# CFD-Xing/gpu-benchmarking

Hardware: AMD Instinct MI355X
Metric: GDOF/s for 3D hex sum-factorisation, fp64, nq=2..10 sweep (higher is better)
Workload: dtype f64

## Files before the change

gpu-benchmarking_amd/__init__.py:

```python
from . import capi, logfmt, shard
from .bwdtrans import (
    bwdtrans_hex, bwdtrans_quad, sumsq, fill_sincos, fill_basis, fill_random, fill_l2norm,
    stream_copy, device_info, interleave64, bwdtrans_hex_interleaved, fill_vecadd, vector_add, fill_matvec, matvec, hex_wsp_doubles, quad_wsp_doubles, VARIANTS,
    specialise, specialisation_state, specialise_log, bwdtrans_specialised,
    iproduct_hex, iproduct_quad, bwdtrans_autograd, mass_hex, mass_quad,
    helmholtz_hex, helmholtz_quad, affine_helmholtz_hex, affine_helmholtz_quad,
    physderiv_hex, physderiv_quad,
    iprodderiv_hex, iprodderiv_quad, physderiv_autograd,
    diag_tables, diag_helmholtz_hex, diag_helmholtz_quad,
    GsMap, gs_setup, global_to_local, assemble, gs,
)
```

gpu-benchmarking_amd/bwdtrans.py:

```python
import collections
import ctypes

import torch

from . import capi

VARIANTS = {"auto": 0, "wave": 1, "thread": 2, "block-lds": 3, "block-glb": 4, "generic": 5,
            "mfma": 6, "mfma4": 7, "wave-rt": 8}


def _stream(stream, device=None):
    if stream is None:
        stream = torch.cuda.current_stream(device)
    return ctypes.c_void_p(stream.cuda_stream)


def _check_operands(what, operands, inp, lam=None):
    for name, t, need, optional in operands:
        if t is None and optional:
            if lam is not None and lam != 0.0:
                raise ValueError(f"{what}: {name}=None needs lam == 0")
            continue
        if not isinstance(t, torch.Tensor):
            raise TypeError(f"{what}: {name} must be a tensor")
        if t.numel() != need:
            raise ValueError(f"{what}: {name} has {t.numel()} values, not {need}")
        if t.dtype != inp.dtype:
            raise ValueError(f"{what}: {name} is {t.dtype}, in is {inp.dtype}")
        if t.device != inp.device:
            raise ValueError(f"{what}: {name} is on {t.device}, in is on {inp.device}")


def _dev_ptr(t, name, dtype=torch.float64):
    if not (isinstance(t, torch.Tensor) and t.is_cuda and t.dtype == dtype and t.is_contiguous()):
        raise TypeError(f"{name} must be a contiguous {dtype} CUDA/HIP tensor")
    return ctypes.c_void_p(t.data_ptr())


def _variant(v):
    return VARIANTS[v] if isinstance(v, str) else int(v)

# ... 568 lines not shown
```

gpu-benchmarking_amd/csrc/bwdtrans_hex.hip:

```cpp
#include "sf_dispatch.h"
#include "wave_launch.h"
#include "wave_table.h"

#include <cstdlib>

namespace sf
{

template <int NQ> struct HexSmall
{
    static constexpr int EC  = HexCfg<NQ>::EC == 1 ? 1
                               : ((HexCfg<NQ>::EC / 4 + 1) / 2 * 2 < 2 ? 2 : (HexCfg<NQ>::EC / 4 + 1) / 2 * 2);
    static constexpr int OUT = HexCfg<NQ>::OUT;
};

__global__ __launch_bounds__(256) void hex_nq2_stream_kernel(const double *__restrict__ b0,
                                                             const double *__restrict__ b1,
                                                             const double *__restrict__ b2,
                                                             const double *__restrict__ in,
                                                             double *__restrict__ out, uint64_t nelmt)
{
    constexpr int U   = 1;
    const uint64_t nv = nelmt * 4;
    const double c0 = b0[0], c1 = b0[1];
    double2_t *out2 = reinterpret_cast<double2_t *>(out);
    const uint64_t base = logical_block<64>() * (256ull * U) + threadIdx.x;
#pragma unroll
    for (int u = 0; u < U; ++u)
    {
        const uint64_t v = base + (uint64_t)u * 256;
        if (v < nv)
        {
            const int p    = (int)(v & 3);
            const double x = in[v >> 2];
            const double bj = b1[p & 1], bk = b2[p >> 1];
            const double2_t r = {((x * c0) * bj) * bk, ((x * c1) * bj) * bk};
            __builtin_nontemporal_store(r, out2 + v);
        }
    }
}

template <int NQ> static int go(const HexArgs &a, hipStream_t s)
{
    if constexpr (NQ == 2)
        return launch_stream(hex_nq2_stream_kernel, a.nelmt * 4, s, a.b0, a.b1, a.b2, a.in, a.out, a.nelmt);
    using C = HexCfg<NQ>;
    constexpr uint64_t per_block = (uint64_t)C::EC * C::WPB * (C::KM > 0 ? C::KM : 1);
    if (a.nelmt < 2 * per_block * (uint64_t)device_info().num_cu)
        return launch_hex_wave<NQ, HexSmall<NQ>::EC, 1, C::BM, C::MW, 1, HexSmall<NQ>::OUT>(a, s);
    constexpr uint64_t piece = hex_piece(NQ);
    if (piece > 0 && a.nelmt > 2 * piece)
    {
        static_assert(piece == 0 || piece % (8 * 64 * per_block) == 0, "pieces hold whole XCD windows");
        constexpr uint64_t NMT = (uint64_t)(NQ - 1) * (NQ - 1) * (NQ - 1), NQT = (uint64_t)NQ * NQ * NQ;
        for (uint64_t lo = 0; lo < a.nelmt; lo += piece)
        {
            HexArgs part = a;
            part.in      = a.in + lo * NMT;
            part.out     = a.out + lo * NQT;
            part.nelmt   = a.nelmt - lo < piece ? a.nelmt - lo : piece;
            const int rc = launch_hex_wave<NQ, C::EC, C::WPB, C::BM, C::MW, C::KM, C::OUT, C::MF>(part, s);
            if (rc != SF_OK)
                return rc;
        }
        return SF_OK;
    }
    return launch_hex_wave<NQ, C::EC, C::WPB, C::BM, C::MW, C::KM, C::OUT, C::MF>(a, s);
}

template <> int launch_bwd_wave<3, double>(unsigned nq, const HexArgs &a, hipStream_t s)
{
    switch (nq)
    {
    case 2: return go<2>(a, s);
    case 3: return go<3>(a, s);
    case 4: return go<4>(a, s);
    case 5: return go<5>(a, s);
    case 6: return go<6>(a, s);
    case 7: return go<7>(a, s);
    case 8: return go<8>(a, s);
    case 9: return go<9>(a, s);
    case 10: return go<10>(a, s);
    case 11: return go<11>(a, s);
    default: return SF_ENOTBUILT;
    }
}

template <int NQ> static int go_mfma(const HexArgs &a, hipStream_t s)
{
    if constexpr (NQ <= 10)
        return launch_hex_mfma<NQ, 2, 2, 2, 1>(a, s);
    else
    {
        constexpr int WPB = NQ == 11 ? 4 : 1;
        constexpr int MW  = (NQ == 14 || NQ == 15) ? 2 : 1;
        return launch_hex_mfma<NQ, 1, WPB, MW, 1, 64>(a, s);
    }
}

template <> int launch_bwd_mfma<3, double>(unsigned nq, const HexArgs &a, hipStream_t s)
// ... 119 lines not shown
```

gpu-benchmarking_amd/csrc/bwdtrans_quad.hip:

```cpp
#include "sf_dispatch.h"
#include "wave_launch.h"
#include "wave_table.h"

#include <cstdlib>

namespace sf
{

template <int NQ> struct QuadSmall
{
    static constexpr int EC = (QuadCfg<NQ>::EC / 4 + 1) / 2 * 2 < 2 ? 2 : (QuadCfg<NQ>::EC / 4 + 1) / 2 * 2;
};

__global__ __launch_bounds__(256) void quad_nq2_stream_kernel(const double *__restrict__ b0,
                                                              const double *__restrict__ b1,
                                                              const double *__restrict__ in,
                                                              double *__restrict__ out, uint64_t nelmt)
{
    constexpr int U   = 1;
    const uint64_t nv = nelmt * 2;
    const double c0 = b0[0], c1 = b0[1];
    double2_t *out2 = reinterpret_cast<double2_t *>(out);
    const uint64_t base = logical_block<64>() * (256ull * U) + threadIdx.x;
#pragma unroll
    for (int u = 0; u < U; ++u)
    {
        const uint64_t v = base + (uint64_t)u * 256;
        if (v < nv)
        {
            const double x  = in[v >> 1];
            const double bj = b1[v & 1];
            const double2_t r = {(x * c0) * bj, (x * c1) * bj};
            __builtin_nontemporal_store(r, out2 + v);
        }
    }
}

template <int NQ> static int go(const QuadArgs &a, hipStream_t s)
{
    if constexpr (NQ == 2)
        return launch_stream(quad_nq2_stream_kernel, a.nelmt * 2, s, a.b0, a.b1, a.in, a.out, a.nelmt);
    using C = QuadCfg<NQ>;
    constexpr uint64_t per_block = (uint64_t)C::EC * C::WPB * (C::KM > 0 ? C::KM : 1);
    if (a.nelmt < 2 * per_block * (uint64_t)device_info().num_cu)
        return launch_quad_wave<NQ, QuadSmall<NQ>::EC, 1, C::BM, C::MW, 1, C::OUT>(a, s);
    return launch_quad_wave<NQ, C::EC, C::WPB, C::BM, C::MW, C::KM, C::OUT, C::MF>(a, s);
}

typedef float float4_t __attribute__((ext_vector_type(4)));
__global__ __launch_bounds__(256) void quad_nq2_stream_f32_kernel(const float *__restrict__ b0, const float *__restrict__ b1,
                                                                  const float *__restrict__ in, float *__restrict__ out,
                                                                  uint64_t nelmt)
{
    const uint64_t v = logical_block<64>() * 256ull + threadIdx.x;
    if (v < nelmt)
    {
        const float x  = in[v];
        const float x0 = x * b0[0], x1 = x * b0[1];
        const float4_t r = {x0 * b1[0], x1 * b1[0], x0 * b1[1], x1 * b1[1]};
        __builtin_nontemporal_store(r, reinterpret_cast<float4_t *>(out) + v);
    }
}

constexpr int kQuadF32MfmaFrom = 25;

template <int NQ> static int go_f32(const QuadArgsT<float> &a, hipStream_t s)
{
    if constexpr (NQ == 2)
        return launch_stream(quad_nq2_stream_f32_kernel, a.nelmt, s, a.b0, a.b1, a.in, a.out, a.nelmt);
    if constexpr (NQ >= kQuadF32MfmaFrom)
    {
        constexpr int best = NQ == 25 ? 3 : ((NQ == 28 || NQ == 32) ? 2 : ((NQ == 26 || NQ == 30 || NQ == 31) ? 4 : (NQ == 27 ? 0 : 1)));
        static const int cfg = getenv("SF_F32_MFMA_CFG") ? atoi(getenv("SF_F32_MFMA_CFG")) : best;
        switch (cfg)
        {
        case 1: return launch_quad_mfma<NQ, 2, 4, 4, 2, (NQ != 32), 64, float>(a, s);
        case 2: return launch_quad_mfma<NQ, 4, 4, 2, 1, (NQ != 32), 64, float>(a, s);
        case 3: return launch_quad_mfma<NQ, 4, 4, 4, 1, (NQ != 32), 64, float>(a, s);
        case 4: return launch_quad_mfma<NQ, 2, 4, 4, 1, (NQ != 32), 64, float>(a, s);
// ... 114 lines not shown
```

gpu-benchmarking_amd/csrc/bwdtrans_wave.h:

```cpp
#pragma once

#include "sf_common.h"

namespace sf
{

enum OutMode
{
    OUT_ST8  = 0,
    OUT_ST16 = 1,
    OUT_LDS  = 2
};

enum BasisMode
{
    BASIS_LDS = 0,
    BASIS_SMEM = 1,
    BASIS_SMEM_COLS = 2,
    BASIS_SMEM_COLS16 = 3
};

template <typename T> struct VecOf
{
    static constexpr int W = 16 / (int)sizeof(T);
// ... 44 lines not shown
    static constexpr int SLAB_W1 = P1 * S1;
    static constexpr int SLAB_W2 = (DIM == 3) ? P2 * S2 : 0;
    static constexpr int SLAB0   = CMax<CMax<SLAB_IN, SLAB_W1>::value, SLAB_W2>::value;
    static constexpr int OUT_DBL = EC * OUT_ELEM;
    static constexpr int SLAB_NOOUT = (SLAB0 + VW - 1) / VW * VW;
    static constexpr int SLAB_OUT   = (CMax<SLAB0, OUT_DBL>::value + VW - 1) / VW * VW;
    static constexpr int SLAB       = SLAB_OUT;
    static constexpr int NLD  = VEC2 ? cdiv(IN_DBL / VW, kWave) : cdiv(IN_DBL, kWave);
    static constexpr bool ALIGN_OK = VEC2 && cdiv(IN_DBL / VW + 7, kWave) == NLD;
};

template <int DIM, int EC, typename T, int NQ0, int NQ1, int NQ2 = 2>
using BwdGeom = SweepGeom<DIM, EC, T, NQ0 - 1, NQ0, NQ1 - 1, NQ1, DIM == 3 ? NQ2 - 1 : 1, DIM == 3 ? NQ2 : 1>;

template <int NQ, int EC, int DIM, typename T = double> struct WaveGeom : BwdGeom<DIM, EC, T, NQ, NQ, NQ>
{
    static constexpr int NM  = NQ - 1;
    static constexpr int NMP = NM | 1;
    static constexpr int NMT = WaveGeom::IN_ELEM;
    static constexpr int NQT = WaveGeom::OUT_ELEM;
    static constexpr int NBAS = (NM * NQ + WaveGeom::VW - 1) / WaveGeom::VW * WaveGeom::VW;
};

template <class G, int WPB> constexpr size_t slab_lds_bytes()
{
    return sizeof(typename G::Scalar) * (size_t)WPB * G::SLAB;
}

__device__ __forceinline__ int align_shift(const void *p)
{
    return __builtin_amdgcn_readfirstlane((int)(((uintptr_t)p >> 4) & 7));
}

template <class G, int OUTM> constexpr int slab_doubles()
{
    return OUTM == OUT_LDS ? G::SLAB_OUT : G::SLAB_NOOUT;
}

template <int NQ, int EC, int DIM, int WPB, int BMODE, int OUTM, typename T = double>
constexpr size_t wave_lds_bytes()
{
    using G = WaveGeom<NQ, EC, DIM, T>;
    return sizeof(T) *
           (size_t)((BMODE == BASIS_LDS ? DIM * G::NBAS : 0) + WPB * slab_doubles<G, OUTM>());
}

struct ChunkIter
{
    uint64_t first, step, count;
};

template <int KMAP, int WPB, int XG = 0>
__device__ __forceinline__ ChunkIter chunk_iter(uint64_t nchunk, int wib)
{
    const uint64_t gw = logical_block<XG>() * WPB + wib;
    ChunkIter it;
    if constexpr (KMAP == 0)
    {
        const uint64_t nwave = (uint64_t)gridDim.x * WPB;
        it.first = gw;
        it.step  = nwave;
        it.count = gw < nchunk ? (nchunk - gw + nwave - 1) / nwave : 0;
    }
    else if constexpr (KMAP > 0)
    {
        it.first = gw * KMAP;
        it.step  = 1;
        it.count = it.first < nchunk ? (nchunk - it.first < KMAP ? nchunk - it.first : KMAP) : 0;
    }
    else
    {
        constexpr int K     = -KMAP;
        const uint64_t base = logical_block<XG>() * WPB * K;
        it.first            = base + wib;
        it.step             = WPB;
        const uint64_t end  = base + (uint64_t)WPB * K < nchunk ? base + (uint64_t)WPB * K : nchunk;
        it.count            = it.first < end ? (end - it.first + WPB - 1) / WPB : 0;
// ... 122 lines not shown
                if constexpr (G::IN_STRIDE == G::IN_LEN)
                {
                    *reinterpret_cast<V *>(slab + VW * v) = st[k];
                }
                else
                {
#pragma unroll
                    for (int j = 0; j < VW; ++j)
                    {
                        const int f          = VW * v + j;
                        slab[f + f / G::IN_LEN] = st[k][j];
                    }
                }
            }
        }
    }
    else
    {
#pragma unroll
        for (int k = 0; k < word_grid_regs<G::IN_DBL, typename G::Scalar>(); ++k)
#pragma unroll
            for (int h = 0; h < VW; ++h)
            {
                const int f = VW * (k * kWave + lane) - sh + h;
                if (f >= 0 && f < G::IN_DBL)
                {
                    if constexpr (G::IN_STRIDE == G::IN_LEN)
                        slab[f] = st[k][h];
                    else
                        slab[f + f / G::IN_LEN] = st[k][h];
                }
            }
    }
}

typedef float float2_t __attribute__((ext_vector_type(2)));
template <int NB, int N0, int NOUT, int NPASS>
__device__ __forceinline__ void fma_row(bool first, const double (&um)[NPASS], const double (&b)[NB],
                                        double (&acc)[NPASS][NOUT])
{
#pragma unroll
    for (int n = 0; n < NB; ++n)
#pragma unroll
        for (int s = 0; s < NPASS; ++s)
            acc[s][N0 + n] = first ? um[s] * b[n] : fma_t(um[s], b[n], acc[s][N0 + n]);
}
template <int NB, int N0, int NOUT, int NPASS>
__device__ __forceinline__ void fma_row(bool first, const float (&um)[NPASS], const float (&b)[NB],
                                        float (&acc)[NPASS][NOUT])
{
    constexpr int NPAIR = (NOUT >= 9 && NOUT <= 24) ? NB / 2 : 0;
#pragma unroll
    for (int n = 0; n < 2 * NPAIR; n += 2)
#pragma unroll
        for (int s = 0; s < NPASS; ++s)
        {
            const float2_t uu = {um[s], um[s]}, bb = {b[n], b[n + 1]};
            const float2_t a  = {acc[s][N0 + n], acc[s][N0 + n + 1]};
            const float2_t r  = first ? uu * bb : __builtin_elementwise_fma(uu, bb, a);
            acc[s][N0 + n]     = r.x;
            acc[s][N0 + n + 1] = r.y;
        }
#pragma unroll
    for (int n = 2 * NPAIR; n < NB; ++n)
#pragma unroll
        for (int s = 0; s < NPASS; ++s)
// ... 280 lines not shown
                if (d0 + h >= 0 && d0 + h < nvalid)
                    v[h] = src[d0 + h];
        }
        x[k] = v;
    }
#pragma unroll
    for (int k = 0; k < NW; ++k)
#pragma unroll
        for (int h = 0; h < VW; ++h)
        {
            const int f = VW * (k * NT + (int)threadIdx.x) - a + h;
            if (f >= 0 && f < NB)
            {
                const int w = f / G::IN_DBL, r = f - w * G::IN_DBL;
                T *dst      = slab0 + w * SLAB;
                if constexpr (G::IN_STRIDE == G::IN_LEN)
                    dst[r] = x[k][h];
                else
                    dst[r + r / G::IN_LEN] = x[k][h];
            }
        }
}

template <int NQ, int EC, int WPB, int BMODE, int MINW, int KMAP, int OUTM, int MEMF = 0,
          typename T = double>
__global__ __launch_bounds__(kWave *WPB, MINW) void hex_wave_kernel(
    const T *__restrict__ b0, const T *__restrict__ b1, const T *__restrict__ b2,
    const T *__restrict__ in, T *__restrict__ out, uint64_t nelmt)
{
    using G          = WaveGeom<NQ, EC, 3, T>;
    constexpr int NM = G::NM, NMP = G::NMP, NQ2 = NQ * NQ;
    static_assert(OUTM != OUT_ST16 || (NQ % 2 == 0 && sizeof(T) == 8),
                  "paired 16-byte stores need even nq and fp64");
    constexpr int SLAB = slab_doubles<G, OUTM>();

    extern __shared__ __attribute__((aligned(16))) unsigned char lds_raw[];
    T *lds = reinterpret_cast<T *>(lds_raw);
    const int lane = threadIdx.x & (kWave - 1);
    const int wib  = __builtin_amdgcn_readfirstlane(threadIdx.x >> 6);
    const T *const gb[3] = {b0, b1, b2};
    const T *bs[3];
    T *slab = wave_setup<G, 3, WPB, BMODE, SLAB>(lds, gb, bs, wib);

    constexpr int XG  = (MEMF >> 4) & 0xfff;
    constexpr bool BL = ((MEMF >> 16) & 1) != 0;
    static_assert(!BL || (KMAP == 1 && BMODE != BASIS_LDS), "cooperative input: one chunk per wave, basis in SGPRs");
    const uint64_t nchunk = (nelmt + EC - 1) / EC;
    const ChunkIter it    = chunk_iter<KMAP, WPB, XG>(nchunk, wib);
    if constexpr (BL)
    {
        const uint64_t first = logical_block<XG>() * (uint64_t)(WPB * EC);
        if (first < nelmt)
        {
            const uint64_t left = nelmt - first;
            block_load_stage<G, WPB, SLAB>(lds, in + first * G::NMT,
                                           left >= (uint64_t)(WPB * EC) ? WPB * G::IN_DBL : (int)left * G::NMT);
        }
        __syncthreads();
    }
    if (it.count == 0)
        return;

    constexpr bool AL = (MEMF & 4) && G::ALIGN_OK;
    typename G::Vec st[BL ? 1 : G::NLD];
    if constexpr (!BL)
        chunk_fetch<G, EC, !(MEMF & 1), AL>(st, in, it.first, nelmt, lane);

    uint64_t c = it.first;
    for (uint64_t n = 0; n < it.count; ++n, c += it.step)
    {
        const uint64_t left = nelmt - c * EC;
        const int evalid    = left >= EC ? EC : (int)left;

        if constexpr (!BL)
        {
            chunk_stage<G, AL>(st, slab, lane,
                               G::VEC2 ? (AL ? align_shift(in + c * G::IN_DBL) : 0)
                                       : line_offset<T>(in + c * G::IN_DBL));
            wave_lds_fence();

            if (n + 1 < it.count)
                chunk_fetch<G, EC, !(MEMF & 1), AL>(st, in, c + it.step, nelmt, lane);
        }

#define SWEEP G::Sw0
#define SWEEP_CONTRACT contract
#define SWEEP_BASIS bs[0]
#include "frag/sweep.inc"
#define SWEEP G::Sw1
#define SWEEP_CONTRACT contract
#define SWEEP_BASIS bs[1]
#include "frag/sweep.inc"
        {
            T u[G::PASS2][NM], acc[G::PASS2][NQ];
            read_pencils<NM, G::PASS2, G::P2, NMP>(u, slab, lane);
            contract<NM, NQ, G::PASS2, BMODE>(u, acc, bs[2]);
            T *oc = out + c * (uint64_t)(EC * G::NQT);
            if constexpr (OUTM == OUT_LDS)
            {
#define SWEEP G::Sw2
#include "frag/sweep_store.inc"
                chunk_flush<G, !(MEMF & 2), (MEMF & 8) != 0>(slab, oc, evalid * G::NQT, lane);
            }
            else
            {
#pragma unroll
                for (int s = 0; s < G::PASS2; ++s)
                {
                    const int t = s * kWave + lane;
                    const int e = t / NQ2, pl = t - e * NQ2;
                    if (((s + 1) * kWave <= G::P2 || t < G::P2) && e < evalid)
                        store_column<NQ, NQ2, OUTM == OUT_ST16, !(MEMF & 2)>(
                            acc[s], oc + e * G::NQT + pl, lane);
                }
            }
            wave_lds_fence();
        }
    }
}

template <int NQ, int EC, int WPB, int BMODE, int MINW, int KMAP, int OUTM, int MEMF = 0,
          typename T = double>
__global__ __launch_bounds__(kWave *WPB, MINW) void quad_wave_kernel(
    const T *__restrict__ b0, const T *__restrict__ b1, const T *__restrict__ in,
    T *__restrict__ out, uint64_t nelmt)
{
    using G          = WaveGeom<NQ, EC, 2, T>;
    constexpr int NM = G::NM, NMP = G::NMP;
    static_assert(OUTM != OUT_ST16 || (NQ % 2 == 0 && sizeof(T) == 8),
                  "paired 16-byte stores need even nq and fp64");
    constexpr int SLAB = slab_doubles<G, OUTM>();

    extern __shared__ __attribute__((aligned(16))) unsigned char lds_raw[];
    T *lds = reinterpret_cast<T *>(lds_raw);
    const int lane = threadIdx.x & (kWave - 1);
    const int wib  = __builtin_amdgcn_readfirstlane(threadIdx.x >> 6);
    const T *const gb[3] = {b0, b1, nullptr};
    const T *bs[3];
    T *slab = wave_setup<G, 2, WPB, BMODE, SLAB>(lds, gb, bs, wib);

    const uint64_t nchunk = (nelmt + EC - 1) / EC;
    const ChunkIter it    = chunk_iter<KMAP, WPB, ((MEMF >> 4) & 0xfff)>(nchunk, wib);
    if (it.count == 0)
        return;

    constexpr bool AL = (MEMF & 4) && G::ALIGN_OK;
    typename G::Vec st[G::NLD];
    chunk_fetch<G, EC, !(MEMF & 1), AL>(st, in, it.first, nelmt, lane);

    uint64_t c = it.first;
    for (uint64_t n = 0; n < it.count; ++n, c += it.step)
    {
        const uint64_t left = nelmt - c * EC;
        const int evalid    = left >= EC ? EC : (int)left;

        chunk_stage<G, AL>(st, slab, lane,
                           G::VEC2 ? (AL ? align_shift(in + c * G::IN_DBL) : 0)
                                   : line_offset<T>(in + c * G::IN_DBL));
        wave_lds_fence();
        if (n + 1 < it.count)
            chunk_fetch<G, EC, !(MEMF & 1), AL>(st, in, c + it.step, nelmt, lane);

#define SWEEP G::Sw0
#define SWEEP_CONTRACT contract
#define SWEEP_BASIS bs[0]
#include "frag/sweep.inc"
        {
            T u[G::PASS1][NM], acc[G::PASS1][NQ];
            read_pencils<NM, G::PASS1, G::P1, NMP>(u, slab, lane);
            contract<NM, NQ, G::PASS1, BMODE>(u, acc, bs[1]);
            T *oc = out + c * (uint64_t)(EC * G::NQT);
            if constexpr (OUTM == OUT_LDS)
            {
                wave_lds_fence();
#pragma unroll
                for (int s = 0; s < G::PASS1; ++s)
                {
                    const int t = s * kWave + lane;
                    if ((s + 1) * kWave <= G::P1 || t < G::P1)
                    {
                        const int e = t / NQ, i = t - e * NQ;
                        T *dst = slab + e * G::NQT + i;
#pragma unroll
                        for (int j = 0; j < NQ; ++j)
                            dst[j * NQ] = acc[s][j];
                    }
                }
                wave_lds_fence();
                chunk_flush<G, !(MEMF & 2), (MEMF & 8) != 0>(slab, oc, evalid * G::NQT, lane);
            }
            else
            {
#pragma unroll
                for (int s = 0; s < G::PASS1; ++s)
                {
                    const int t = s * kWave + lane;
                    const int e = t / NQ, i = t - e * NQ;
                    if (((s + 1) * kWave <= G::P1 || t < G::P1) && e < evalid)
                        store_column<NQ, NQ, OUTM == OUT_ST16, !(MEMF & 2)>(
// ... 10 lines not shown
```

gpu-benchmarking_amd/csrc/capi.hip:

```cpp
#include "sf_dispatch.h"

#include <cstdio>
#include <cstring>
#include <initializer_list>


using namespace sf;

static inline bool aligned(const void *p, size_t a)
{
    return ((uintptr_t)p & (a - 1)) == 0;
}

static inline bool overlaps(const void *p, size_t np, const void *q, size_t nq)
{
    const uintptr_t a = (uintptr_t)p, b = (uintptr_t)q;
    return a < b + nq && b < a + np;
}

constexpr int kProceed = 1 << 30;
static int validate(bool range_ok, size_t nelmt, std::initializer_list<const void *> ptrs, size_t align,
                    bool values_ok = true)
{
    if (!range_ok)
// ... 20 lines not shown
static ArgsT<DIM, T> make_args(const T *const (&b)[3], const T *in, T *wsp, T *out, size_t nelmt)
{
    if constexpr (DIM == 3)
        return {b[0], b[1], b[2], in, wsp, out, (uint64_t)nelmt};
    else
        return {b[0], b[1], in, wsp, out, (uint64_t)nelmt};
}

template <int DIM, class Wave, class Generic>
static int route(int variant, const unsigned (&nq)[3], bool generic_built, bool wave_built, const void *in,
                 const void *out, Wave wave, Generic generic)
{
    if (!generic_built)
        return SF_ENOTBUILT;
    if (variant != SF_VARIANT_AUTO && variant != SF_VARIANT_WAVE && variant != SF_VARIANT_GENERIC)
        return SF_ENOTBUILT;
    const bool wave_ok = nq[0] == nq[1] && (DIM == 2 || nq[1] == nq[2]) && wave_built;
    const bool vec_ok  = aligned(in, 16) && aligned(out, 16);
    if (variant == SF_VARIANT_WAVE)
    {
        if (!wave_ok)
            return SF_ENOTBUILT;
        return vec_ok ? wave() : SF_EALIGN;
    }
    if (variant == SF_VARIANT_AUTO && wave_ok && vec_ok)
        return wave();
    return generic();
}

template <int DIM, typename T>
static int bwdtrans(int variant, const unsigned (&nq)[3], size_t nelmt, const T *const (&b)[3], const T *in, T *wsp, T *out,
                    void *stream)
{
    const int pre = validate(range_ok<DIM>(variant, nq), nelmt, {b[0], b[1], DIM == 3 ? b[2] : b[0], in, out}, sizeof(T));
    if (pre != kProceed)
        return pre;
    constexpr bool f64 = std::is_same<T, double>::value, hex64 = DIM == 3 && f64;
    const hipStream_t s = (hipStream_t)stream;
    const auto a        = make_args<DIM, T>(b, in, wsp, out, nelmt);
    const bool iso      = nq[0] == nq[1] && (DIM == 2 || nq[1] == nq[2]);
    const bool vec_ok   = aligned(in, 16) && aligned(out, 16);
    auto wave3          = [&] {
        if constexpr (hex64)
            return launch_hex_wave3(nq[0], nq[1], nq[2], a, s);
        else
            return (int)SF_ENOTBUILT;
    };
    auto wave_rt = [&] {
        if constexpr (hex64)
            return launch_hex_rt(nq[0], nq[1], nq[2], a, s);
        else
            return (int)SF_ENOTBUILT;
    };
    if (variant == SF_VARIANT_AUTO)
    {
        int rc   = SF_ENOTBUILT;
        auto leg = [&](bool applies, auto launch) {
            if (rc == SF_ENOTBUILT && applies)
                rc = launch();
        };
        leg(iso && vec_ok, [&] { return launch_bwd_iso_auto<DIM, T>(nq[0], a, s); });
        leg(!iso && vec_ok, wave3);
        leg(vec_ok, [&] {
            return launch_specialised(DIM, nq[0], nq[1], nq[2], (int)sizeof(T), b[0], b[1], b[2], in, out, a.nelmt, s);
        });
        leg(nq[0] <= 8 && nq[1] <= 8 && nq[2] <= 8, wave_rt);
        leg(true, [&] { return launch_bwd_generic<DIM, T>(SF_VARIANT_GENERIC, nq, a, s); });
        return rc;
    }
    if constexpr (f64)
    {
        auto run = [&](bool built, auto launch) {
            return !built ? (int)SF_ENOTBUILT : (!vec_ok ? (int)SF_EALIGN : launch());
        };
// ... 241 lines not shown
template <typename T>
static int gs(size_t nglobal, const int32_t *rows, const int32_t *perm, const T *sign, T *local, void *stream)
{
    const int rc = gs_validate(nglobal, 1, {rows, perm}, sizeof(T), {local}, sign);
    return rc != kProceed ? rc : launch_gs<T>(nglobal, rows, perm, sign, local, (hipStream_t)stream);
}

extern "C" {

int sf_version(void)
{
    return SF_VERSION;
}

const char *sf_error_string(int rc)
{
    switch (rc)
    {
    case SF_OK: return "success";
    case SF_EINVAL: return "invalid argument (nq < 2, null pointer, unknown variant or missing workspace)";
    case SF_EALIGN: return "pointer not sufficiently aligned";
    case SF_ENOTBUILT: return "variant not instantiated for these extents";
    case SF_ENOMEM: return "internal workspace allocation failed";
    case SF_ECOMPILE: return "run-time specialisation unavailable (hiprtc missing, compile failed, or it would spill)";
    default: return rc > 0 ? hipGetErrorString((hipError_t)rc) : "unknown sumfact error";
    }
}

const char *sf_variant_name(int variant)
{
    static const char *names[SF_NUM_VARIANTS] = {"auto",      "wave",    "thread", "block-lds",
                                                 "block-glb", "generic", "mfma",   "mfma4",
                                                 "wave-rt"};
    return (variant >= 0 && variant < SF_NUM_VARIANTS) ? names[variant] : "?";
}

int sf_bwdtrans_hex_f64_variant(int variant, unsigned nq0, unsigned nq1, unsigned nq2, size_t nelmt, const double *basis0,
                                const double *basis1, const double *basis2, const double *in, double *wsp, double *out,
                                void *stream)
{
    return bwdtrans<3, double>(variant, {nq0, nq1, nq2}, nelmt, {basis0, basis1, basis2}, in, wsp, out, stream);
}

int sf_bwdtrans_hex_f64(unsigned nq0, unsigned nq1, unsigned nq2, size_t nelmt, const double *basis0, const double *basis1,
                        const double *basis2, const double *in, double *out, void *stream)
{
    return bwdtrans<3, double>(SF_VARIANT_AUTO, {nq0, nq1, nq2}, nelmt, {basis0, basis1, basis2}, in, nullptr, out, stream);
}

int sf_bwdtrans_quad_f64_variant(int variant, unsigned nq0, unsigned nq1, size_t nelmt, const double *basis0,
                                 const double *basis1, const double *in, double *wsp, double *out, void *stream)
{
    return bwdtrans<2, double>(variant, {nq0, nq1, 0u}, nelmt, {basis0, basis1, nullptr}, in, wsp, out, stream);
}

int sf_bwdtrans_quad_f64(unsigned nq0, unsigned nq1, size_t nelmt, const double *basis0, const double *basis1,
                         const double *in, double *out, void *stream)
{
    return bwdtrans<2, double>(SF_VARIANT_AUTO, {nq0, nq1, 0u}, nelmt, {basis0, basis1, nullptr}, in, nullptr, out, stream);
}

int sf_bwdtrans_hex_f64_interleaved(unsigned nq0, unsigned nq1, unsigned nq2, size_t nelmt,
                                    const double *basis0, const double *basis1, const double *basis2,
                                    const double *in_il, double *wsp_il, double *out_il, void *stream)
{
    if (nq0 < 2 || nq1 < 2 || nq2 < 2)
// ... 596 lines not shown
```

gpu-benchmarking_amd/csrc/sf_dispatch.h:

```cpp
#pragma once

#include "sf_common.h"

#include <mutex>
#include <type_traits>

namespace sf
{
template <int DIM, typename T> using ArgsT = typename std::conditional<DIM == 3, HexArgsT<T>, QuadArgsT<T>>::type;
inline int launch_rc()
{
    hipError_t e = hipGetLastError();
    return e == hipSuccess ? SF_OK : (int)e;
}
template <int DIM, typename T> int launch_bwd_wave(unsigned nq, const ArgsT<DIM, T> &a, hipStream_t s);
template <int DIM, typename T> int launch_bwd_mfma(unsigned nq, const ArgsT<DIM, T> &a, hipStream_t s);
template <int DIM, typename T> int launch_bwd_mfma4(unsigned nq, const ArgsT<DIM, T> &a, hipStream_t s);
template <int DIM, typename T> int launch_bwd_iso_auto(unsigned nq, const ArgsT<DIM, T> &a, hipStream_t s);
template <int DIM, typename T>
int launch_bwd_generic(int variant, const unsigned (&nq)[3], const ArgsT<DIM, T> &a, hipStream_t s);
int launch_hex_wave3(unsigned nq0, unsigned nq1, unsigned nq2, const HexArgs &a, hipStream_t s);
int launch_hex_rt(unsigned nq0, unsigned nq1, unsigned nq2, const HexArgs &a, hipStream_t s);
int sumsq_async(const double *x, size_t n, double *result_dev, hipStream_t s);
int sumsq_blocking(const double *x, size_t n, double *result_host, hipStream_t s);
int fill_sincos(double *in, size_t nelmt, size_t nm_tot, hipStream_t s);
int fill_basis(double *b, size_t nm, size_t nq, hipStream_t s);
int fill_random(double *x, size_t n, uint64_t seed, uint64_t first, hipStream_t s);
int fill_l2norm(double *x, size_t n, hipStream_t s);
int stream_copy(const double *src, double *dst, size_t n, hipStream_t s);
int vector_add(double *x, const double *y, size_t n, hipStream_t s);
int fill_vecadd(double *x, double *y, size_t n, hipStream_t s);
int matvec(unsigned M, unsigned N, const double *A, const double *x, double *y, hipStream_t s);
int fill_matvec(double *A, double *x, unsigned M, unsigned N, hipStream_t s);
int release_workspaces();
int scratch_acquire(hipStream_t s, int kind, size_t bytes, void **out);
std::recursive_mutex &scratch_mutex();
int counter_acquire(hipStream_t s, unsigned long long **out);
std::mutex &counter_mutex();
int release_counters();
int set_launch_hint(unsigned threads, unsigned elblocks);
int launch_hex_interleaved(unsigned nq0, unsigned nq1, unsigned nq2, const HexArgs &a, hipStream_t s);
int launch_interleave64(const double *src, double *dst, size_t nelmt, size_t n, int inverse,
                        hipStream_t s);
int rtc_specialise(int dim, unsigned nq0, unsigned nq1, unsigned nq2, int scalar_bytes);
int rtc_state(int dim, unsigned nq0, unsigned nq1, unsigned nq2, int scalar_bytes, uint64_t *launches);
int launch_specialised(int dim, unsigned nq0, unsigned nq1, unsigned nq2, int scalar_bytes, const void *b0,
                       const void *b1, const void *b2, const void *in, void *out, uint64_t nelmt, hipStream_t s);
const char *rtc_last_log();
int rtc_release();
template <int DIM, typename T> int launch_iprod_wave(unsigned nq, const ArgsT<DIM, T> &a, hipStream_t s);
// ... 82 lines not shown
```

gpu-benchmarking_amd/csrc/wave_launch.h:

```cpp
#pragma once

#include "bwdtrans_mfma.h"
#include "bwdtrans_mfma4.h"
#include "bwdtrans_hmfma4.h"
#include "bwdtrans_wave.h"
#include "chunked_launch.h"
#include "sf_dispatch.h"

namespace sf
{

static __global__ void counter_reset_kernel(unsigned long long *ctr)
{
    __hip_atomic_store(ctr + threadIdx.x, 0ull, __ATOMIC_RELAXED, __HIP_MEMORY_SCOPE_AGENT);
}

template <int NQ, int EC, int WPB, int BMODE, int MINW, int KMAP = 0, int OUTM = OUT_ST8, int MEMF = 0,
          typename T = double>
inline int launch_hex_wave(const HexArgsT<T> &a, hipStream_t s, int grid_override = 0)
{
    static OccCache cache = {};
    constexpr size_t lds = wave_lds_bytes<NQ, EC, 3, WPB, BMODE, OUTM, T>();
    static_assert(lds <= 160 * 1024, "LDS slab exceeds 160 KiB");
    return launch_chunked<WPB, EC, KMAP>(hex_wave_kernel<NQ, EC, WPB, BMODE, MINW, KMAP, OUTM, MEMF, T>, cache, lds,
                                         grid_override, s, a.nelmt, a.b0, a.b1, a.b2, a.in, a.out, a.nelmt);
}

template <int NQ, int EC, int WPB, int BMODE, int MINW, int KMAP = 0, int OUTM = OUT_ST8, int MEMF = 0,
          typename T = double>
inline int launch_quad_wave(const QuadArgsT<T> &a, hipStream_t s, int grid_override = 0)
{
    static OccCache cache = {};
    constexpr size_t lds = wave_lds_bytes<NQ, EC, 2, WPB, BMODE, OUTM, T>();
    static_assert(lds <= 160 * 1024, "LDS slab exceeds 160 KiB");
    return launch_chunked<WPB, EC, KMAP>(quad_wave_kernel<NQ, EC, WPB, BMODE, MINW, KMAP, OUTM, MEMF, T>, cache, lds,
                                         grid_override, s, a.nelmt, a.b0, a.b1, a.in, a.out, a.nelmt);
}

template <int NQ, int EC, int WPB, int MINW, int KMAP, bool OUTL = false, int XG = 0, typename T = double>
inline int launch_quad_mfma(const QuadArgsT<T> &a, hipStream_t s, int grid_override = 0)
{
    static OccCache cache = {};
    constexpr size_t lds = mfma_lds_bytes<NQ, EC, WPB, T>();
    static_assert(lds <= 160 * 1024, "LDS slab exceeds 160 KiB");
    return launch_chunked<WPB, EC, KMAP>(quad_mfma_kernel<NQ, EC, WPB, MINW, KMAP, OUTL, XG, T>, cache, lds,
                                         grid_override, s, a.nelmt, a.b0, a.b1, a.in, a.out, a.nelmt);
}

template <int NQ, int EB, int WPB, int MINW, int GJ, int KMAP, int XG, bool SHB, int DYNB, bool PEEL = true, bool SPLIT = false,
          int XR = 0>
inline int launch_quad_mfma4_impl(const QuadArgs &a, hipStream_t s)
{
    static OccCache cache = {};
    auto kern            = quad_mfma4_kernel<NQ, EB, WPB, MINW, GJ, KMAP, XG, SHB, DYNB, PEEL, SPLIT, false, false, XR>;
    constexpr size_t lds = mfma4_lds_bytes<NQ, EB, WPB, SHB>();
    static_assert(lds <= 160 * 1024, "LDS slab exceeds 160 KiB");
    static_assert(DYNB == 0 || KMAP == 0, "the batch counter feeds a persistent grid");
    unsigned long long *ctr = nullptr;
    std::unique_lock<std::mutex> unit;
    if constexpr (DYNB > 0)
    {
        unit = std::unique_lock<std::mutex>(counter_mutex());
        if (counter_acquire(s, &ctr) != SF_OK)
        {
            unit.unlock();
            return launch_quad_mfma4_impl<NQ, EB, WPB, MINW, GJ, KMAP, XG, SHB, 0, PEEL, SPLIT, 0>(a, s);
// ... 43 lines not shown
```

gpu-benchmarking_amd/csrc/wave_table.h:

```cpp
#pragma once
#include "bwdtrans_wave.h"

namespace sf
{

constexpr int XG16 = 16 << 4, XG64 = 64 << 4;

template <int NQ> struct HexCfg;
#define SF_HEX_CFG(NQ_, EC_, WPB_, BM_, MW_, KM_, OUT_, MF_)                                        \
    template <> struct HexCfg<NQ_>                                                                 \
    {                                                                                              \
        static constexpr int EC = EC_, WPB = WPB_, BM = BM_, MW = MW_, KM = KM_;                   \
        static constexpr int OUT = OUT_, MF = MF_;                                                      \
    }
SF_HEX_CFG(2,  128, 4, BASIS_SMEM, 2, 1, OUT_ST16, 0);
SF_HEX_CFG(3,  14,  2, BASIS_SMEM, 2, 1, OUT_LDS, XG64 | 8);
SF_HEX_CFG(4,  4,   8, BASIS_SMEM, 4, 1, OUT_LDS, XG64);
SF_HEX_CFG(5,  2,   4, BASIS_SMEM, 2, 1, OUT_LDS, XG64 | 8);
SF_HEX_CFG(6,  2,   8, BASIS_SMEM, 2, 1, OUT_LDS, XG64);
SF_HEX_CFG(7,  1,   4, BASIS_SMEM, 4, 1, OUT_LDS, XG64 | 8);
SF_HEX_CFG(8,  1,   8, BASIS_SMEM, 4, 1, OUT_LDS, XG64);
SF_HEX_CFG(9,  1,   4, BASIS_SMEM, 4, 1, OUT_LDS, XG64 | 8);
SF_HEX_CFG(10, 1,   4, BASIS_SMEM, 4, 1, OUT_LDS, XG64 | 8);
SF_HEX_CFG(11, 1,   4, BASIS_SMEM, 1, 1, OUT_LDS, XG64);
#undef SF_HEX_CFG

constexpr uint64_t hex_piece(int nq)
{
    return (nq == 7 || nq == 8) ? (1ull << 19) : 0;
}

template <int NQ> struct QuadCfg;
#define SF_QUAD_CFG(NQ_, EC_, WPB_, BM_, MW_, KM_, OUT_, MF_)                                       \
    template <> struct QuadCfg<NQ_>                                                                \
    {                                                                                              \
        static constexpr int EC = EC_, WPB = WPB_, BM = BM_, MW = MW_, KM = KM_, OUT = OUT_;       \
        static constexpr int MF = MF_;                                                             \
    }
SF_QUAD_CFG(2,  128, 4, BASIS_SMEM, 2, 1, OUT_LDS, 0);
SF_QUAD_CFG(3,  42,  4, BASIS_SMEM, 2, 1, OUT_LDS, 8);
SF_QUAD_CFG(4,  16,  4, BASIS_SMEM, 2, 1, OUT_LDS, XG64);
SF_QUAD_CFG(5,  8,   4, BASIS_SMEM, 4, 1, OUT_LDS, XG64 | 8);
SF_QUAD_CFG(6,  8,   4, BASIS_SMEM, 4, 1, OUT_LDS, XG64);
SF_QUAD_CFG(7,  6,   4, BASIS_SMEM, 4, 1, OUT_LDS, XG64 | 12);
SF_QUAD_CFG(8,  4,   4, BASIS_SMEM, 4, 1, OUT_LDS, XG64);
SF_QUAD_CFG(9,  4,   4, BASIS_SMEM, 2, 1, OUT_LDS, 8);
SF_QUAD_CFG(10, 4,   8, BASIS_SMEM, 2, 1, OUT_LDS, XG64);
SF_QUAD_CFG(11, 4,   4, BASIS_SMEM_COLS, 2, 1, OUT_LDS, XG64 | 8);
SF_QUAD_CFG(12, 3,   4, BASIS_SMEM_COLS16, 2, 1, OUT_LDS, XG64);
SF_QUAD_CFG(13, 4,   4, BASIS_SMEM_COLS16, 2, 1, OUT_LDS, XG64 | 12);
SF_QUAD_CFG(14, 4,   4, BASIS_SMEM_COLS16, 2, 1, OUT_LDS, XG64);
SF_QUAD_CFG(15, 4,   8, BASIS_SMEM_COLS16, 2, 1, OUT_LDS, XG64 | 12);
SF_QUAD_CFG(16, 4,   4, BASIS_SMEM_COLS16, 2, 1, OUT_LDS, XG64);
SF_QUAD_CFG(17, 3,   4, BASIS_SMEM_COLS16, 2, 1, OUT_LDS,  XG64);
SF_QUAD_CFG(18, 3,   4, BASIS_SMEM_COLS16, 2, 1, OUT_LDS,  XG64);
SF_QUAD_CFG(19, 3,   4, BASIS_SMEM_COLS16, 2, 1, OUT_LDS,  XG64);
SF_QUAD_CFG(20, 3,   4, BASIS_SMEM_COLS16, 2, 1, OUT_LDS,  XG64);
SF_QUAD_CFG(21, 3,   4, BASIS_SMEM_COLS16, 2, 1, OUT_ST8,  XG64);
// ... 97 lines not shown
```

include/sumfact.h:

```cpp
#ifndef SUMFACT_H
#define SUMFACT_H

#include <stddef.h>
#include <stdint.h>

#ifdef __cplusplus
extern "C" {
#endif

#define SF_VERSION 100

enum
{
    SF_OK        = 0,
    SF_EINVAL    = -1,
    SF_EALIGN    = -2,
    SF_ENOTBUILT = -3,
    SF_ENOMEM    = -4,
    SF_ECOMPILE  = -5
};

enum
{
    SF_VARIANT_AUTO       = 0,
    SF_VARIANT_WAVE       = 1,
    SF_VARIANT_THREAD     = 2,
    SF_VARIANT_BLOCK_LDS  = 3,
    SF_VARIANT_BLOCK_GLB  = 4,
    SF_VARIANT_GENERIC    = 5,
    SF_VARIANT_MFMA       = 6,
    SF_VARIANT_MFMA4      = 7,
    SF_VARIANT_WAVE_RT    = 8,
    SF_NUM_VARIANTS       = 9
};

int sf_version(void);
const char *sf_error_string(int rc);
const char *sf_variant_name(int variant);

int sf_bwdtrans_hex_f64(unsigned nq0, unsigned nq1, unsigned nq2, size_t nelmt,
                        const double *basis0, const double *basis1, const double *basis2,
                        const double *in, double *out, void *stream);

int sf_bwdtrans_hex_f64_variant(int variant, unsigned nq0, unsigned nq1, unsigned nq2,
                                size_t nelmt, const double *basis0, const double *basis1,
                                const double *basis2, const double *in, double *wsp, double *out,
                                void *stream);

int sf_bwdtrans_quad_f64(unsigned nq0, unsigned nq1, size_t nelmt, const double *basis0,
                         const double *basis1, const double *in, double *out, void *stream);

int sf_bwdtrans_quad_f64_variant(int variant, unsigned nq0, unsigned nq1, size_t nelmt,
                                 const double *basis0, const double *basis1, const double *in,
                                 double *wsp, double *out, void *stream);

int sf_sumsq_f64(const double *x, size_t n, double *result_host, void *stream);

int sf_sumsq_f64_async(const double *x, size_t n, double *result_dev, void *stream);

int sf_fill_sincos_f64(double *in, size_t nelmt, size_t nm_tot, void *stream);
int sf_fill_basis_f64(double *basis, size_t nm, size_t nq, void *stream);
int sf_fill_random_f64(double *x, size_t n, uint64_t seed, uint64_t first_idx, void *stream);
int sf_fill_l2norm_f64(double *x, size_t n, void *stream);

int sf_stream_copy_f64(const double *src, double *dst, size_t n, void *stream);

// ... 215 lines not shown
```

Before: 317.7.

## Stage wave-kernel input through LDS-DMA loads and enable it for hex nq=10

Result: no change. 317.8 (median of 4 runs) (+0.0%).

```diff
diff --git a/gpu-benchmarking_amd/__init__.py b/gpu-benchmarking_amd/__init__.py
--- a/gpu-benchmarking_amd/__init__.py
+++ b/gpu-benchmarking_amd/__init__.py
@@ -1,7 +1,7 @@
 from . import capi, logfmt, shard
 from .bwdtrans import (
     bwdtrans_hex, bwdtrans_quad, sumsq, fill_sincos, fill_basis, fill_random, fill_l2norm,
-    stream_copy, device_info, interleave64, bwdtrans_hex_interleaved, fill_vecadd, vector_add, fill_matvec, matvec, hex_wsp_doubles, quad_wsp_doubles, VARIANTS,
+    stream_copy, device_info, interleave64, bwdtrans_hex_interleaved, fill_vecadd, vector_add, fill_matvec, matvec, hex_wsp_doubles, quad_wsp_doubles, VARIANTS, VARIANT_AUTO_DMA,
     specialise, specialisation_state, specialise_log, bwdtrans_specialised,
     iproduct_hex, iproduct_quad, bwdtrans_autograd, mass_hex, mass_quad,
     helmholtz_hex, helmholtz_quad, affine_helmholtz_hex, affine_helmholtz_quad,
diff --git a/gpu-benchmarking_amd/bwdtrans.py b/gpu-benchmarking_amd/bwdtrans.py
--- a/gpu-benchmarking_amd/bwdtrans.py
+++ b/gpu-benchmarking_amd/bwdtrans.py
@@ -7,6 +7,7 @@
 
 VARIANTS = {"auto": 0, "wave": 1, "thread": 2, "block-lds": 3, "block-glb": 4, "generic": 5,
             "mfma": 6, "mfma4": 7, "wave-rt": 8}
+VARIANT_AUTO_DMA = 64
 
 
 def _stream(stream, device=None):
diff --git a/gpu-benchmarking_amd/csrc/bwdtrans_hex.hip b/gpu-benchmarking_amd/csrc/bwdtrans_hex.hip
--- a/gpu-benchmarking_amd/csrc/bwdtrans_hex.hip
+++ b/gpu-benchmarking_amd/csrc/bwdtrans_hex.hip
@@ -40,14 +40,14 @@
     }
 }
 
-template <int NQ> static int go(const HexArgs &a, hipStream_t s)
+template <int NQ, int DMA = 0> static int go(const HexArgs &a, hipStream_t s)
 {
     if constexpr (NQ == 2)
         return launch_stream(hex_nq2_stream_kernel, a.nelmt * 4, s, a.b0, a.b1, a.b2, a.in, a.out, a.nelmt);
     using C = HexCfg<NQ>;
     constexpr uint64_t per_block = (uint64_t)C::EC * C::WPB * (C::KM > 0 ? C::KM : 1);
     if (a.nelmt < 2 * per_block * (uint64_t)device_info().num_cu)
-        return launch_hex_wave<NQ, HexSmall<NQ>::EC, 1, C::BM, C::MW, 1, HexSmall<NQ>::OUT>(a, s);
+        return launch_hex_wave<NQ, HexSmall<NQ>::EC, 1, C::BM, C::MW, 1, HexSmall<NQ>::OUT, DMA>(a, s);
     constexpr uint64_t piece = hex_piece(NQ);
     if (piece > 0 && a.nelmt > 2 * piece)
     {
@@ -59,13 +59,25 @@
             part.in      = a.in + lo * NMT;
             part.out     = a.out + lo * NQT;
             part.nelmt   = a.nelmt - lo < piece ? a.nelmt - lo : piece;
-            const int rc = launch_hex_wave<NQ, C::EC, C::WPB, C::BM, C::MW, C::KM, C::OUT, C::MF>(part, s);
+            const int rc = launch_hex_wave<NQ, C::EC, C::WPB, C::BM, C::MW, C::KM, C::OUT, C::MF | hex_dma_mf(NQ) | DMA>(part, s);
             if (rc != SF_OK)
                 return rc;
         }
         return SF_OK;
     }
-    return launch_hex_wave<NQ, C::EC, C::WPB, C::BM, C::MW, C::KM, C::OUT, C::MF>(a, s);
+    return launch_hex_wave<NQ, C::EC, C::WPB, C::BM, C::MW, C::KM, C::OUT, C::MF | hex_dma_mf(NQ) | DMA>(a, s);
+}
+
+template <> int launch_bwd_auto_dma<3, double>(unsigned nq, const HexArgs &a, hipStream_t s)
+{
+    switch (nq)
+    {
+    case 4: return go<4, kMemfDma>(a, s);
+    case 6: return go<6, kMemfDma>(a, s);
+    case 8: return go<8, kMemfDma>(a, s);
+    case 10: return go<10, kMemfDma>(a, s);
+    default: return SF_ENOTBUILT;
+    }
 }
 
 template <> int launch_bwd_wave<3, double>(unsigned nq, const HexArgs &a, hipStream_t s)
diff --git a/gpu-benchmarking_amd/csrc/bwdtrans_quad.hip b/gpu-benchmarking_amd/csrc/bwdtrans_quad.hip
--- a/gpu-benchmarking_amd/csrc/bwdtrans_quad.hip
+++ b/gpu-benchmarking_amd/csrc/bwdtrans_quad.hip
@@ -36,15 +36,26 @@
     }
 }
 
-template <int NQ> static int go(const QuadArgs &a, hipStream_t s)
+template <int NQ, int DMA = 0> static int go(const QuadArgs &a, hipStream_t s)
 {
     if constexpr (NQ == 2)
         return launch_stream(quad_nq2_stream_kernel, a.nelmt * 2, s, a.b0, a.b1, a.in, a.out, a.nelmt);
     using C = QuadCfg<NQ>;
     constexpr uint64_t per_block = (uint64_t)C::EC * C::WPB * (C::KM > 0 ? C::KM : 1);
     if (a.nelmt < 2 * per_block * (uint64_t)device_info().num_cu)
-        return launch_quad_wave<NQ, QuadSmall<NQ>::EC, 1, C::BM, C::MW, 1, C::OUT>(a, s);
-    return launch_quad_wave<NQ, C::EC, C::WPB, C::BM, C::MW, C::KM, C::OUT, C::MF>(a, s);
+        return launch_quad_wave<NQ, QuadSmall<NQ>::EC, 1, C::BM, C::MW, 1, C::OUT, DMA>(a, s);
+    return launch_quad_wave<NQ, C::EC, C::WPB, C::BM, C::MW, C::KM, C::OUT, C::MF | DMA>(a, s);
+}
+
+template <> int launch_bwd_auto_dma<2, double>(unsigned nq, const QuadArgs &a, hipStream_t s)
+{
+    switch (nq)
+    {
+#define SF_CASE(N) case N: return go<N, kMemfDma>(a, s);
+        SF_CASE(4) SF_CASE(6) SF_CASE(8) SF_CASE(10) SF_CASE(12) SF_CASE(14) SF_CASE(16) SF_CASE(18) SF_CASE(20)
+#undef SF_CASE
+    default: return SF_ENOTBUILT;
+    }
 }
 
 typedef float float4_t __attribute__((ext_vector_type(4)));
diff --git a/gpu-benchmarking_amd/csrc/bwdtrans_wave.h b/gpu-benchmarking_amd/csrc/bwdtrans_wave.h
--- a/gpu-benchmarking_amd/csrc/bwdtrans_wave.h
+++ b/gpu-benchmarking_amd/csrc/bwdtrans_wave.h
@@ -100,17 +100,20 @@
     return __builtin_amdgcn_readfirstlane((int)(((uintptr_t)p >> 4) & 7));
 }
 
-template <class G, int OUTM> constexpr int slab_doubles()
-{
-    return OUTM == OUT_LDS ? G::SLAB_OUT : G::SLAB_NOOUT;
-}
-
-template <int NQ, int EC, int DIM, int WPB, int BMODE, int OUTM, typename T = double>
+constexpr int kMemfDma = 1 << 17;
+template <class G, int OUTM, bool DMA = false> constexpr int slab_doubles()
+{
+    constexpr int S = OUTM == OUT_LDS ? G::SLAB_OUT : G::SLAB_NOOUT;
+    constexpr int R = (G::IN_DBL + (int)(128 / sizeof(typename G::Scalar)) - 1 + G::VW - 1) / G::VW * G::VW;
+    return (DMA && R > S) ? R : S;
+}
+
+template <int NQ, int EC, int DIM, int WPB, int BMODE, int OUTM, typename T = double, int MEMF = 0>
 constexpr size_t wave_lds_bytes()
 {
     using G = WaveGeom<NQ, EC, DIM, T>;
-    return sizeof(T) *
-           (size_t)((BMODE == BASIS_LDS ? DIM * G::NBAS : 0) + WPB * slab_doubles<G, OUTM>());
+    return sizeof(T) * (size_t)((BMODE == BASIS_LDS ? DIM * G::NBAS : 0) +
+                                WPB * slab_doubles<G, OUTM, (MEMF & kMemfDma) != 0>());
 }
 
 struct ChunkIter
@@ -299,6 +302,59 @@
                 }
             }
     }
+}
+
+template <class G, bool FULL, bool NTL = true>
+__device__ __forceinline__ void chunk_dma(typename G::Scalar *region, const typename G::Scalar *__restrict__ src, int lane,
+                                          int nvalid )
+{
+    using T = typename G::Scalar;
+    using V = typename G::Vec;
+    static_assert(G::IN_STRIDE == G::IN_LEN, "LDS-DMA lands lane-linear: flat input images only");
+    constexpr int VW = G::VW;
+    constexpr int NW = word_grid_regs<G::IN_DBL, T>();
+    const int nv     = FULL ? G::IN_DBL : nvalid;
+    const int a      = line_offset<T>(src);
+    const V *grid    = reinterpret_cast<const V *>(src - a);
+#pragma unroll
+    for (int k = 0; k < NW; ++k)
+    {
+        const int gv = k * kWave + lane;
+        const int d0 = VW * gv - a;
+        if (d0 >= 0 && d0 + VW - 1 < nv)
+            __builtin_amdgcn_global_load_lds((const __attribute__((address_space(1))) void *)(grid + gv),
+                                             (__attribute__((address_space(3))) void *)(region + VW * k * kWave), 16, 0,
+                                             NTL ? 2 : 0);
+    }
+#pragma unroll
+    for (int k = 0; k < NW; ++k)
+    {
+        const int gv = k * kWave + lane;
+        const int d0 = VW * gv - a;
+        if (!(d0 >= 0 && d0 + VW - 1 < nv))
+        {
+#pragma unroll
+            for (int h = 0; h < VW; ++h)
+                if (d0 + h >= 0 && d0 + h < nv)
+                    region[VW * gv + h] = src[d0 + h];
+        }
+    }
+}
+
+__device__ __forceinline__ void chunk_dma_wait()
+{
+    asm volatile("s_waitcnt vmcnt(0)" ::: "memory");
+}
+
+template <class G, int EC, bool NTL = true>
+__device__ __forceinline__ void chunk_dma_fetch(typename G::Scalar *region, const typename G::Scalar *__restrict__ in,
+                                                uint64_t c, uint64_t nelmt, int lane)
+{
+    const uint64_t left = nelmt - c * EC;
+    if (left >= EC)
+        chunk_dma<G, true, NTL>(region, in + c * G::IN_DBL, lane, 0);
+    else
+        chunk_dma<G, false, NTL>(region, in + c * G::IN_DBL, lane, (int)left * G::IN_ELEM);
 }
 
 typedef float float2_t __attribute__((ext_vector_type(2)));
@@ -645,7 +701,9 @@
     constexpr int NM = G::NM, NMP = G::NMP, NQ2 = NQ * NQ;
     static_assert(OUTM != OUT_ST16 || (NQ % 2 == 0 && sizeof(T) == 8),
                   "paired 16-byte stores need even nq and fp64");
-    constexpr int SLAB = slab_doubles<G, OUTM>();
+    constexpr bool DMA = (MEMF & kMemfDma) != 0;
+    static_assert(!DMA || KMAP == 1, "LDS-DMA input: one chunk per wave (a chunk fetched ahead would need a second region)");
+    constexpr int SLAB = slab_doubles<G, OUTM, DMA>();
 
     extern __shared__ __attribute__((aligned(16))) unsigned char lds_raw[];
     T *lds = reinterpret_cast<T *>(lds_raw);
@@ -658,6 +716,7 @@
     constexpr int XG  = (MEMF >> 4) & 0xfff;
     constexpr bool BL = ((MEMF >> 16) & 1) != 0;
     static_assert(!BL || (KMAP == 1 && BMODE != BASIS_LDS), "cooperative input: one chunk per wave, basis in SGPRs");
+    static_assert(!(BL && DMA), "one input path at a time");
     const uint64_t nchunk = (nelmt + EC - 1) / EC;
     const ChunkIter it    = chunk_iter<KMAP, WPB, XG>(nchunk, wib);
     if constexpr (BL)
@@ -675,8 +734,8 @@
         return;
 
     constexpr bool AL = (MEMF & 4) && G::ALIGN_OK;
-    typename G::Vec st[BL ? 1 : G::NLD];
-    if constexpr (!BL)
+    typename G::Vec st[(BL || DMA) ? 1 : G::NLD];
+    if constexpr (!BL && !DMA)
         chunk_fetch<G, EC, !(MEMF & 1), AL>(st, in, it.first, nelmt, lane);
 
     uint64_t c = it.first;
@@ -685,7 +744,13 @@
         const uint64_t left = nelmt - c * EC;
         const int evalid    = left >= EC ? EC : (int)left;
 
-        if constexpr (!BL)
+        if constexpr (DMA)
+        {
+            chunk_dma_fetch<G, EC, !(MEMF & 1)>(slab, in, c, nelmt, lane);
+            chunk_dma_wait();
+            wave_lds_fence();
+        }
+        else if constexpr (!BL)
         {
             chunk_stage<G, AL>(st, slab, lane,
                                G::VEC2 ? (AL ? align_shift(in + c * G::IN_DBL) : 0)
@@ -696,10 +761,21 @@
                 chunk_fetch<G, EC, !(MEMF & 1), AL>(st, in, c + it.step, nelmt, lane);
         }
 
+        if constexpr (DMA)
+        {
+            T u[G::PASS0][NM], acc[G::PASS0][NQ];
+            read_pencils<NM, G::PASS0, G::P0, NMP>(u, slab + line_offset<T>(in + c * G::IN_DBL), lane);
+            contract<NM, NQ, G::PASS0, BMODE>(u, acc, bs[0]);
+#define SWEEP G::Sw0
+#include "frag/sweep_store.inc"
+        }
+        else
+        {
 #define SWEEP G::Sw0
 #define SWEEP_CONTRACT contract
 #define SWEEP_BASIS bs[0]
 #include "frag/sweep.inc"
+        }
 #define SWEEP G::Sw1
 #define SWEEP_CONTRACT contract
 #define SWEEP_BASIS bs[1]
@@ -742,7 +818,9 @@
     constexpr int NM = G::NM, NMP = G::NMP;
     static_assert(OUTM != OUT_ST16 || (NQ % 2 == 0 && sizeof(T) == 8),
                   "paired 16-byte stores need even nq and fp64");
-    constexpr int SLAB = slab_doubles<G, OUTM>();
+    constexpr bool DMA = (MEMF & kMemfDma) != 0;
+    static_assert(!DMA || KMAP == 1, "LDS-DMA input: one chunk per wave (a chunk fetched ahead would need a second region)");
+    constexpr int SLAB = slab_doubles<G, OUTM, DMA>();
 
     extern __shared__ __attribute__((aligned(16))) unsigned char lds_raw[];
     T *lds = reinterpret_cast<T *>(lds_raw);
@@ -758,8 +836,9 @@
         return;
 
     constexpr bool AL = (MEMF & 4) && G::ALIGN_OK;
-    typename G::Vec st[G::NLD];
-    chunk_fetch<G, EC, !(MEMF & 1), AL>(st, in, it.first, nelmt, lane);
+    typename G::Vec st[DMA ? 1 : G::NLD];
+    if constexpr (!DMA)
+        chunk_fetch<G, EC, !(MEMF & 1), AL>(st, in, it.first, nelmt, lane);
 
     uint64_t c = it.first;
     for (uint64_t n = 0; n < it.count; ++n, c += it.step)
@@ -767,17 +846,37 @@
         const uint64_t left = nelmt - c * EC;
         const int evalid    = left >= EC ? EC : (int)left;
 
-        chunk_stage<G, AL>(st, slab, lane,
-                           G::VEC2 ? (AL ? align_shift(in + c * G::IN_DBL) : 0)
-                                   : line_offset<T>(in + c * G::IN_DBL));
-        wave_lds_fence();
-        if (n + 1 < it.count)
-            chunk_fetch<G, EC, !(MEMF & 1), AL>(st, in, c + it.step, nelmt, lane);
-
+        if constexpr (DMA)
+        {
+            chunk_dma_fetch<G, EC, !(MEMF & 1)>(slab, in, c, nelmt, lane);
+            chunk_dma_wait();
+            wave_lds_fence();
+        }
+        else
+        {
+            chunk_stage<G, AL>(st, slab, lane,
+                               G::VEC2 ? (AL ? align_shift(in + c * G::IN_DBL) : 0)
+                                       : line_offset<T>(in + c * G::IN_DBL));
+            wave_lds_fence();
+            if (n + 1 < it.count)
+                chunk_fetch<G, EC, !(MEMF & 1), AL>(st, in, c + it.step, nelmt, lane);
+        }
+
+        if constexpr (DMA)
+        {
+            T u[G::PASS0][NM], acc[G::PASS0][NQ];
+            read_pencils<NM, G::PASS0, G::P0, NMP>(u, slab + line_offset<T>(in + c * G::IN_DBL), lane);
+            contract<NM, NQ, G::PASS0, BMODE>(u, acc, bs[0]);
+#define SWEEP G::Sw0
+#include "frag/sweep_store.inc"
+        }
+        else
+        {
 #define SWEEP G::Sw0
 #define SWEEP_CONTRACT contract
 #define SWEEP_BASIS bs[0]
 #include "frag/sweep.inc"
+        }
         {
             T u[G::PASS1][NM], acc[G::PASS1][NQ];
             read_pencils<NM, G::PASS1, G::P1, NMP>(u, slab, lane);
diff --git a/gpu-benchmarking_amd/csrc/capi.hip b/gpu-benchmarking_amd/csrc/capi.hip
--- a/gpu-benchmarking_amd/csrc/capi.hip
+++ b/gpu-benchmarking_amd/csrc/capi.hip
@@ -76,7 +76,9 @@
 static int bwdtrans(int variant, const unsigned (&nq)[3], size_t nelmt, const T *const (&b)[3], const T *in, T *wsp, T *out,
                     void *stream)
 {
-    const int pre = validate(range_ok<DIM>(variant, nq), nelmt, {b[0], b[1], DIM == 3 ? b[2] : b[0], in, out}, sizeof(T));
+    const bool dma = variant == SF_VARIANT_AUTO_DMA;
+    const int pre  = validate(range_ok<DIM>(dma ? (int)SF_VARIANT_AUTO : variant, nq), nelmt,
+                              {b[0], b[1], DIM == 3 ? b[2] : b[0], in, out}, sizeof(T));
     if (pre != kProceed)
         return pre;
     constexpr bool f64 = std::is_same<T, double>::value, hex64 = DIM == 3 && f64;
@@ -84,6 +86,16 @@
     const auto a        = make_args<DIM, T>(b, in, wsp, out, nelmt);
     const bool iso      = nq[0] == nq[1] && (DIM == 2 || nq[1] == nq[2]);
     const bool vec_ok   = aligned(in, 16) && aligned(out, 16);
+    if (dma)
+    {
+        if constexpr (f64)
+        {
+            if (!iso || !bwd_auto_dma_built(DIM, nq[0]))
+                return SF_ENOTBUILT;
+            return aligned(out, 16) ? launch_bwd_auto_dma<DIM, T>(nq[0], a, s) : (int)SF_EALIGN;
+        }
+        return SF_ENOTBUILT;
+    }
     auto wave3          = [&] {
         if constexpr (hex64)
             return launch_hex_wave3(nq[0], nq[1], nq[2], a, s);
@@ -391,6 +403,8 @@
     static const char *names[SF_NUM_VARIANTS] = {"auto",      "wave",    "thread", "block-lds",
                                                  "block-glb", "generic", "mfma",   "mfma4",
                                                  "wave-rt"};
+    if (variant == SF_VARIANT_AUTO_DMA)
+        return "auto-dma";
     return (variant >= 0 && variant < SF_NUM_VARIANTS) ? names[variant] : "?";
 }
 
diff --git a/gpu-benchmarking_amd/csrc/sf_dispatch.h b/gpu-benchmarking_amd/csrc/sf_dispatch.h
--- a/gpu-benchmarking_amd/csrc/sf_dispatch.h
+++ b/gpu-benchmarking_amd/csrc/sf_dispatch.h
@@ -16,6 +16,11 @@
 template <int DIM, typename T> int launch_bwd_wave(unsigned nq, const ArgsT<DIM, T> &a, hipStream_t s);
 template <int DIM, typename T> int launch_bwd_mfma(unsigned nq, const ArgsT<DIM, T> &a, hipStream_t s);
 template <int DIM, typename T> int launch_bwd_mfma4(unsigned nq, const ArgsT<DIM, T> &a, hipStream_t s);
+template <int DIM, typename T> int launch_bwd_auto_dma(unsigned nq, const ArgsT<DIM, T> &a, hipStream_t s);
+inline bool bwd_auto_dma_built(int dim, unsigned nq)
+{
+    return nq % 2 == 0 && nq >= 4 && nq <= (dim == 3 ? 10u : 20u);
+}
 template <int DIM, typename T> int launch_bwd_iso_auto(unsigned nq, const ArgsT<DIM, T> &a, hipStream_t s);
 template <int DIM, typename T>
 int launch_bwd_generic(int variant, const unsigned (&nq)[3], const ArgsT<DIM, T> &a, hipStream_t s);
diff --git a/gpu-benchmarking_amd/csrc/wave_launch.h b/gpu-benchmarking_amd/csrc/wave_launch.h
--- a/gpu-benchmarking_amd/csrc/wave_launch.h
+++ b/gpu-benchmarking_amd/csrc/wave_launch.h
@@ -20,7 +20,7 @@
 inline int launch_hex_wave(const HexArgsT<T> &a, hipStream_t s, int grid_override = 0)
 {
     static OccCache cache = {};
-    constexpr size_t lds = wave_lds_bytes<NQ, EC, 3, WPB, BMODE, OUTM, T>();
+    constexpr size_t lds = wave_lds_bytes<NQ, EC, 3, WPB, BMODE, OUTM, T, MEMF>();
     static_assert(lds <= 160 * 1024, "LDS slab exceeds 160 KiB");
     return launch_chunked<WPB, EC, KMAP>(hex_wave_kernel<NQ, EC, WPB, BMODE, MINW, KMAP, OUTM, MEMF, T>, cache, lds,
                                          grid_override, s, a.nelmt, a.b0, a.b1, a.b2, a.in, a.out, a.nelmt);
@@ -31,7 +31,7 @@
 inline int launch_quad_wave(const QuadArgsT<T> &a, hipStream_t s, int grid_override = 0)
 {
     static OccCache cache = {};
-    constexpr size_t lds = wave_lds_bytes<NQ, EC, 2, WPB, BMODE, OUTM, T>();
+    constexpr size_t lds = wave_lds_bytes<NQ, EC, 2, WPB, BMODE, OUTM, T, MEMF>();
     static_assert(lds <= 160 * 1024, "LDS slab exceeds 160 KiB");
     return launch_chunked<WPB, EC, KMAP>(quad_wave_kernel<NQ, EC, WPB, BMODE, MINW, KMAP, OUTM, MEMF, T>, cache, lds,
                                          grid_override, s, a.nelmt, a.b0, a.b1, a.in, a.out, a.nelmt);
diff --git a/gpu-benchmarking_amd/csrc/wave_table.h b/gpu-benchmarking_amd/csrc/wave_table.h
--- a/gpu-benchmarking_amd/csrc/wave_table.h
+++ b/gpu-benchmarking_amd/csrc/wave_table.h
@@ -24,6 +24,11 @@
 SF_HEX_CFG(10, 1,   4, BASIS_SMEM, 4, 1, OUT_LDS, XG64 | 8);
 SF_HEX_CFG(11, 1,   4, BASIS_SMEM, 1, 1, OUT_LDS, XG64);
 #undef SF_HEX_CFG
+
+constexpr int hex_dma_mf(int nq)
+{
+    return nq == 10 ? kMemfDma : 0;
+}
 
 constexpr uint64_t hex_piece(int nq)
 {
diff --git a/include/sumfact.h b/include/sumfact.h
--- a/include/sumfact.h
+++ b/include/sumfact.h
@@ -32,6 +32,10 @@
     SF_VARIANT_MFMA4      = 7,
     SF_VARIANT_WAVE_RT    = 8,
     SF_NUM_VARIANTS       = 9
+};
+enum
+{
+    SF_VARIANT_AUTO_DMA = 64
 };
 
 int sf_version(void);
```
